# christopher-beckham/gan-heightmaps

Hardware: AMD Instinct MI355X
Metric: 512px heightmap+texture train images/sec (higher is better)
Workload: dtype bf16x3; 1 GPU; test1_nobn_bilin_both joint DCGAN+pix2pix train step (train_mode=both), 512x512, batch 4 per GPU, RMSprop lr 1e-4, LSGAN+100*L1; fp32 by operand splitting on the bf16 matrix cores (3 exact bf16 pieces per operand, 6 products, fp32 accumulation); global_batch=4, in_shp=512, parallelism=dp1, hip_graph=False, issue=recorded, streams=3

## Files before the change

gan_heightmaps_amd/_lib.py:

```python
import ctypes as C
import os

_HERE = os.path.dirname(os.path.abspath(__file__))
LIB_PATH = os.path.join(_HERE, "libghm.so")


class GhmError(RuntimeError):
    pass


class ConvDesc(C.Structure):
    _fields_ = [("N", C.c_int32), ("C", C.c_int32), ("H", C.c_int32), ("W", C.c_int32),
                ("K", C.c_int32), ("Ho", C.c_int32), ("Wo", C.c_int32),
                ("kh", C.c_int32), ("kw", C.c_int32), ("stride", C.c_int32), ("pad", C.c_int32),
                ("x_nstride", C.c_int64), ("y_nstride", C.c_int64)]


class RenderParams(C.Structure):
    _fields_ = [("pos", C.c_float * 3), ("yaw", C.c_float), ("pitch", C.c_float), ("fov", C.c_float),
                ("Hi", C.c_int32), ("Wi", C.c_int32),
                ("height_scale", C.c_float), ("step", C.c_float), ("max_dist", C.c_float),
                ("sun_azimuth", C.c_float), ("sun_elevation", C.c_float), ("shadows", C.c_int32),
                ("softness", C.c_float), ("ambient", C.c_float), ("haze", C.c_float),
                ("horizon", C.c_float * 3), ("zenith", C.c_float * 3), ("accel", C.c_int32), ("out_u8", C.c_int32)]
# ... 116 lines not shown
    "ghm_maxpool2_fwd": [_p, _p, _p, _i32, _i32, _i32, _i32],
    "ghm_maxpool2_bwd": [_p, _p, _p, _p, _p, _i32, _i32, _i32, _i32, _i32, _f],
    "ghm_avgpool_fwd": [_p, _p, _p, _i32, _i32, _i32, _i32, _i32],
    "ghm_avgpool_bwd": [_p, _p, _p, _i32, _i32, _i32, _i32, _i32],
    "ghm_dropout": [_p, _p, _i64, _p, _i64, _i32, _i32, _i32, _f, C.c_uint32, _p],
    "ghm_counter_tick": [_p, _p],
    "ghm_transpose_weights_batched": [_p, _p, _i32, _i32],
    "ghm_upconv_collapse_weights": [_p, _p, _p, _p, _p, _i32, _i32],
    "ghm_upconv_collapse_batched": [_p, _p, _i32, _i32],
    "ghm_upconv_expand_batched": [_p, _p, _i32, _i32, _i32],
    "ghm_blconv_frame_sizes": [_i32, _i32, _i32, _i32, _i32, C.POINTER(_i64), C.POINTER(_i64)],
    "ghm_blconv_frame_fwd": [_p, _p, _i64, _p, _p, _i64, _i32, _i32, _i32, _i32, _i32, _p],
    "ghm_blconv_frame_gather": [_p, _p, _i64, _i32, _i32, _i32, _i32, _i32, _p],
    "ghm_blconv_frame_dgrad": [_p, _p, _p, _p, _i64, _i32, _i32, _i32, _i32, _i32],
    "ghm_blconv_frame_wgrad": [_p, _p, _p, _p, _i32, _i32, _i32, _i32, _i32],
    "ghm_blconv_fwd_split": [_p, _D, _p, _i64, _i64, _p, _p, _p, _i32],
    "ghm_blconv_dgrad_split": [_p, _D, _p, _i64, _i64, _p, _p, _i32, _i32],
    "ghm_blconv_wgrad_split": [_p, _D, _p, _i64, _i64, _p, _i64, _i64, _p, _p, _i32, _i32],
    "ghm_upconv_expand_wgrad": [_p, _p, _p, _i32, _i32, _i32],
    "ghm_pp_to_hi": [_p, _p, _p, _i64, _i32, _i32, _i32, _i32],
    "ghm_hi_to_pp": [_p, _p, _i64, _p, _i32, _i32, _i32, _i32],
    "ghm_upsample_nearest2_fwd": [_p, _p, _i64, _p, _i32, _i32, _i32, _i32],
    "ghm_upsample_nearest2_bwd": [_p, _p, _p, _i64, _i32, _i32, _i32, _i32, _i32],
    "ghm_upsample_bilinear2_fwd": [_p, _p, _i64, _p, _i32, _i32, _i32, _i32],
    "ghm_upsample_bilinear2_bwd": [_p, _p, _p, _i64, _i32, _i32, _i32, _i32, _i32],
    "ghm_copy_view": [_p, _p, _i64, _p, _i64, _i32, _i32, _i32, _i32],
    "ghm_scale_samples": [_p, _p, _i64, _i32, _i32, _i32, _p, _i64, _p, _i64],
    "ghm_axpby": [_p, _f, _p, _f, _p, _i64],
    "ghm_image_batch": [_p, _p, _i32, _i32, _i32, _i32, _p, _i32, _p, _i64],
    "ghm_texture_gather": [_p, _p, _i32, _i32, _i32, _i32, _i32, _i32, _i32, _i32, _i32, _i32, _i32, _i32, _i32, _p, _i64],
# ... 128 lines not shown
```

gan_heightmaps_amd/csrc/conv_split.hip:

```cpp
#include <stdlib.h>
#include <string.h>

#include "common.h"

namespace {

typedef float f32x16 __attribute__((ext_vector_type(16)));
typedef float f32x2 __attribute__((ext_vector_type(2)));
typedef unsigned u32x4 __attribute__((ext_vector_type(4)));
typedef __bf16 bf16x8 __attribute__((ext_vector_type(8)));
typedef __bf16 bf16x2 __attribute__((ext_vector_type(2)));

__device__ __forceinline__ f32x16 sp_mfma(u32x4 a, u32x4 b, f32x16 c) {
    return __builtin_amdgcn_mfma_f32_32x32x16_bf16(__builtin_bit_cast(bf16x8, a), __builtin_bit_cast(bf16x8, b), c, 0, 0, 0);
}

__device__ __forceinline__ void sp_split2(float a, float b, unsigned& p0, unsigned& p1, unsigned& p2) {
    f32x2 v = {a, b};
    p0 = __builtin_bit_cast(unsigned, __builtin_convertvector(v, bf16x2));
    f32x2 r = {a - __uint_as_float(p0 << 16), b - __uint_as_float(p0 & 0xffff0000u)};
    p1 = __builtin_bit_cast(unsigned, __builtin_convertvector(r, bf16x2));
    f32x2 r2 = {r[0] - __uint_as_float(p1 << 16), r[1] - __uint_as_float(p1 & 0xffff0000u)};
    p2 = __builtin_bit_cast(unsigned, __builtin_convertvector(r2, bf16x2));
}
// ... 264 lines not shown
    static constexpr int PU1 = 2 * PH * PW, PCH = (PU1 + 63) / 64, PUP = PCH * 64;
    static constexpr int WU1 = 2 * KS * BM, NI = WU1 / 64;
    static constexpr int NW = WM * WN;
    static constexpr int NQ = (PCH + NW - 1) / NW;
    static constexpr int NIW = (NP * NI + NW - 1) / NW;
    static constexpr int WUNITS = NP * WU1, PUNITS = NP * PUP;
    static constexpr int SCR = 2 * WUNITS + 2 * PUNITS;
    static constexpr int LDS_BYTES = (SCR + 64 + 32) * 16;
};

template <int V>
struct SpIC {
    static constexpr int value = V;
};

template <int KS, int ST, int BM, int RT, int WM, int WN, bool POOL, int TW, int NP, int ABL = 0, int CLS = 0>
__global__ __launch_bounds__(WM * WN * 64, 1) void sp_conv2_kernel(const SpConvArgs a) {
    static_assert(CLS == 0 || (KS == 3 && ST == 1 && !POOL && ABL == 0), "class forms: 3x3 stride 1");
    typedef SpGeo2<KS, ST, BM, RT, WM, WN, TW, NP> G;
    typedef SpProd<NP> PR;
    constexpr int T = KS * KS;
    constexpr int RPF = G::RPF, ROWS = G::ROWS;
    constexpr int TM = BM / (WM * 32), TN = RT / WN;
    constexpr int PH = G::PH, PW = G::PW, PU1 = G::PU1, PCH = G::PCH, PUP = G::PUP;
    constexpr int PWE = (PW + 1) / 2;
    constexpr int WU1 = G::WU1, NI = G::NI, NW = G::NW, NQ = G::NQ, NIW = G::NIW;
    constexpr int WUNITS = G::WUNITS, PUNITS = G::PUNITS, SCR = G::SCR;
    constexpr int NMF = PR::N * TM * TN;
    constexpr int NRD = NP * (TM + TN);
    static_assert(TM >= 1 && TN >= 1 && KS >= 3, "tile / pipeline shape");
    extern __shared__ __attribute__((aligned(16))) u32x4 sp_smem[];
// ... 2 lines not shown
    u32x4* const Bl = sp_smem + SCR + 64;

    const int tid = threadIdx.x, lane = tid & 63, wave = __builtin_amdgcn_readfirstlane(tid >> 6);
    const int wm = wave / WN, wn = wave % WN;
    const int kg = lane >> 5, li = lane & 31;
    const int ntr = (a.R + BM - 1) / BM;
    const int tiles_x = a.W / TW, tiles_y = a.H / ROWS;
    const int lx = li % TW, ly = li / TW;
    const int HW = a.H * a.W, HWin = a.Hin * a.Win;
    const int nslabs = a.CH / 16;
    const int s_begin = blockIdx.y * a.slabs_per_split;
    const int s_end = min(nslabs, s_begin + a.slabs_per_split);
    struct Tile {
        int r0, n, y0, x0;
    };
    auto decode = [&](int v) {
        int L = CLS == 1 ? v : sp_xcd_remap(v, a.ntiles);
        Tile t;
        if (CLS == 1) {
            const int gs = a.cls_group, span = ntr * gs;
            const int g = L / span, rem = L - g * span;
            t.r0 = (rem / gs) * BM;
            L = g * gs + rem % gs;
        } else {
            t.r0 = (L % ntr) * BM;
            L /= ntr;
        }
        const int tx = L % tiles_x;
        L /= tiles_x;
        const int ty = L % tiles_y;
        t.n = L / tiles_y;
        t.y0 = ty * ROWS;
        t.x0 = tx * TW;
        return t;
    };
    int v = blockIdx.x;
    Tile tc = decode(v);
    const int cls1 = CLS == 1 ? tc.r0 / a.cls_k : 0;
    const int fa0 = CLS == 1 ? (cls1 >> 1) : 0, b0 = CLS == 1 ? (cls1 & 1) : 0;

    typedef const __attribute__((address_space(1))) void* gptr_t;
    typedef __attribute__((address_space(3))) void* lptr_t;

    const unsigned lane16 = lane * 16;
    unsigned wu[NIW];
    int wl[NIW];
    bool wreal[NIW];
    int wcol[NIW];
#pragma unroll
    for (int i = 0; i < NIW; ++i) {
        const int j = wave + i * NW;
        wreal[i] = j < NP * NI;
        const int jj = wreal[i] ? j : 0;
        const int p = jj / NI, w = jj - p * NI;
        const int ci = w / (BM / 64), h = w - ci * (BM / 64);
        const int cb = ci / KS, b = ci - cb * KS;
        wu[i] = (unsigned)(((long)p * a.wq_pstride + ((long)cb * T + b) * a.Rpad + h * 64) * 16);
        wl[i] = p * WU1 + w * 64;
        wcol[i] = b;
        if (CLS == 1 && b < b0) wreal[i] = false;
    }
    const long wrow = (long)KS * a.Rpad * 16;
    const long wslab = (long)2 * T * a.Rpad * 16;
    auto dma_w = [&](int r0, int s, int fa, int tog, int nc = KS) {
        const char* const src = (const char*)(a.wq + r0) + (long)s * wslab + fa * wrow;
#pragma unroll
        for (int i = 0; i < NIW; ++i)
            if (CLS != 0) {
                const bool real = wreal[i] && (CLS != 2 || wcol[i] < nc);
                __builtin_amdgcn_global_load_lds(real ? (gptr_t)(src + wu[i] + lane16) : (gptr_t)a.zeros,
                                                 (lptr_t)(sp_smem + (real ? wl[i] + tog : SCR)), 16, 0, 0);
            } else if (ABL & 16)
                __builtin_amdgcn_global_load_lds((gptr_t)(src + wu[i] + lane16), (lptr_t)(sp_smem + (wreal[i] ? wl[i] + tog : SCR)), 4, 0, 0);
            else if (ABL & 8)
                __builtin_amdgcn_global_load_lds((gptr_t)a.zeros, (lptr_t)(sp_smem + (wreal[i] ? wl[i] + tog : SCR)), 16, 0, 0);
            else
                __builtin_amdgcn_global_load_lds((gptr_t)(src + wu[i] + lane16), (lptr_t)(sp_smem + (wreal[i] ? wl[i] + tog : SCR)), 16, 0, 0);
    };

    const char* pp[NQ];
    unsigned pok = 0;
    int pcb[NQ], pyx[NQ];
    int pl[NQ];
    bool preal[NQ];
// ... 35 lines not shown
                    __builtin_amdgcn_global_load_lds((gptr_t)g, (lptr_t)(sp_smem + (preal[q] ? 2 * WUNITS + tog + p * PUP + pl[q] : SCR)), 4, 0, 0);
                else if (ABL & 8)
                    __builtin_amdgcn_global_load_lds((gptr_t)a.zeros, (lptr_t)(sp_smem + (preal[q] ? 2 * WUNITS + tog + p * PUP + pl[q] : SCR)), 16, 0, 0);
                else
                    __builtin_amdgcn_global_load_lds((gptr_t)g, (lptr_t)(sp_smem + (preal[q] ? 2 * WUNITS + tog + p * PUP + pl[q] : SCR)), 16, 0, 0);
                g += ok ? pstep : 0;
            }
        }
    };

    f32x16 acc[TM][TN], accc[TM][TN];

    struct Frag {
        u32x4 a[NP][TM], b[NP][TN];
    };
    const int wlane = kg * KS * BM + wm * (BM / WM) + li + b0 * BM;
    const int plane = kg * PH * PW + ((wn * TN * RPF + ly) * ST) * PW + (ST == 2 ? lx : lx * ST) + fa0 * PW + b0;
    auto rd = [&](Frag& f, const u32x4* Wb, const u32x4* Pb, int fa, int b) {
#pragma unroll
        for (int p = 0; p < NP; ++p) {
#pragma unroll
            for (int i = 0; i < TM; ++i) f.a[NP - 1 - p][i] = Wb[(NP - 1 - p) * WU1 + b * BM + i * 32];
#pragma unroll
            for (int j = 0; j < TN; ++j)
                f.b[p][j] = Pb[p * PUP + fa * PW + j * RPF * ST * PW + (ST == 2 ? (b & 1) * PWE + (b >> 1) : b)];
        }
    };
    auto mm = [&](const Frag& f) {
#pragma unroll
        for (int pr = 0; pr < PR::N; ++pr) {
#pragma unroll
            for (int i = 0; i < TM; ++i)
#pragma unroll
                for (int j = 0; j < TN; ++j) {
                    if (pr < PR::N - 1)
                        accc[i][j] = sp_mfma(f.a[PR::A[pr]][i], f.b[PR::B[pr]][j], accc[i][j]);
                    else
                        acc[i][j] = sp_mfma(f.a[0][i], f.b[0][j], acc[i][j]);
                }
        }
    };

    const int s_last = s_end - 1;
    auto ncols_of = [&](int s) { return CLS == 2 ? 3 - ((s / (a.cls_k / 16)) & 1) : KS; };
    if (s_begin < s_end) {
        dma_w(tc.r0, s_begin, fa0, 0, ncols_of(s_begin));
        dma_p(0, false);
    }
    asm volatile("s_waitcnt vmcnt(0)\n\ts_barrier" ::: "memory");
    if (s_begin < s_end) dma_w(tc.r0, s_begin, fa0 + 1, WUNITS, ncols_of(s_begin));
    int w0 = 0, p0 = 0;
    Frag cur;
    rd(cur, Wl + wlane, Pl + plane, 0, 0);

    for (;;) {
        const int vn = v + gridDim.x;
        const bool more = NW == 4 && CLS == 0 && vn < a.ntiles && s_begin < s_end;
        const Tile tn = decode(more ? vn : v);
#pragma unroll
        for (int i = 0; i < TM; ++i)
#pragma unroll
            for (int j = 0; j < TN; ++j)
#pragma unroll
                for (int e = 0; e < 16; ++e) acc[i][j][e] = accc[i][j][e] = 0.f;

        auto run = [&](auto NR_, auto NC_, int s_lo, int s_hi) {
            constexpr int NR = decltype(NR_)::value, NC = decltype(NC_)::value;
            static_assert(NR >= 2 && NC >= 2, "at least two filter rows / columns per slab");
            for (int s = s_lo; s < s_hi; ++s) {
                const bool last = s == s_last;
                const int sn = last ? (more ? s_begin : s) : s + 1;
                const int rn = (last && more) ? tn.r0 : tc.r0;
                const u32x4* const Pc = Pl + p0 + plane;
                const u32x4* const Pn = Pl + (PUNITS - p0) + plane;
#pragma unroll
                for (int fa = 0; fa < NR; ++fa) {
                    const int wc = (fa & 1) ? WUNITS - w0 : w0;
                    const u32x4* const Wc = Wl + wc + wlane;
                    const u32x4* const Wn = Wl + (WUNITS - wc) + wlane;
#pragma unroll
                    for (int b = 0; b < NC; ++b) {
                        Frag nx;
                        int ndma = 0;
                        if (ABL & 4) {
                            nx = cur;
                        } else if (b + 1 < NC) {
                            rd(nx, Wc, Pc, fa, b + 1);
                        } else {
                            rd(nx, Wn, fa + 1 < NR ? Pc : Pn, fa + 1 < NR ? fa + 1 : 0, 0);
                        }
                        if (b + 1 == NC && !(ABL & 1)) {
                            if (fa + 2 < NR)
                                dma_w(tc.r0, s, fa0 + fa + 2, wc, NC);
                            else
                                dma_w(rn, sn, fa0 + fa + 2 - NR, wc, ncols_of(sn));
                            ndma = NIW;
                        }
                        if (fa == 0 && b == 0 && !(ABL & 1)) {
                            if (last && more)
                                patch_of(tn);
                            dma_p(PUNITS - p0, !last);
                            ndma = NP * NQ;
                        }
                        mm(cur);
#pragma unroll
                        for (int m_ = 0; m_ < NRD; ++m_) {
                            __builtin_amdgcn_sched_group_barrier(0x008, 1, 0);
                            __builtin_amdgcn_sched_group_barrier(0x100, 1, 0);
                        }
#pragma unroll
// ... 24 lines not shown
                case 2: run(SpIC<2>{}, SpIC<3>{}, s_begin, s_end); break;
                default: run(SpIC<2>{}, SpIC<2>{}, s_begin, s_end); break;
            }
        } else {
            const int spc = a.cls_k / 16;
            run(SpIC<3>{}, SpIC<3>{}, max(s_begin, 0), min(s_end, spc));
            run(SpIC<3>{}, SpIC<2>{}, max(s_begin, spc), min(s_end, 2 * spc));
            run(SpIC<2>{}, SpIC<3>{}, max(s_begin, 2 * spc), min(s_end, 3 * spc));
            run(SpIC<2>{}, SpIC<2>{}, max(s_begin, 3 * spc), min(s_end, 4 * spc));
        }

        sp_conv_epilogue<BM, RT, WM, WN, POOL, TW, TM, TN, NP>(a, acc, accc, Bl, tid, wm, wn, kg, li, lx, ly, tc.n, tc.r0, tc.y0, tc.x0, HW);
        if (!more) break;
        v = vn;
        tc = tn;
    }
    asm volatile("s_waitcnt vmcnt(0)" ::: "memory");
}

struct SpWgradArgs {
    const u32x4* xq;
    long xq_ns, xq_ps;
    const u32x4* dyq;
    long dyq_ns, dyq_ps;
    const u32x4* zeros;
    float* out;
    int N, C, H, W, K, Ho, Wo;
    int rows_per_split, splits_per_col;
    long split_stride;
    int accumulate;
// ... 960 lines not shown
    for (int i = 0; i < nseen; ++i)
        if (seen[i] == (const void*)kernel) return 0;
    GHM_HIP(hipFuncSetAttribute((const void*)kernel, hipFuncAttributeMaxDynamicSharedMemorySize, 160 * 1024));
    if (nseen < 64) seen[nseen++] = (const void*)kernel;
    return 0;
}

template <int KS, int ST, int BM, int RT, int WM, int WN, bool POOL, int TW>
int sp_launch_variant(ghm_ctx* ctx, dim3 g, size_t lds, const SpConvArgs& a, int np, int cls = 0) {
    static_assert(SpGeo2<KS, ST, BM, RT, WM, WN, TW, 3>::LDS_BYTES <= 160 * 1024, "LDS");
    if (cls) {
        if constexpr (KS == 3 && ST == 1 && !POOL && TW == 32) {
#define GHM_CLS_CASE(NP_, C_)                                                                                                     \
            if constexpr (BM == 64 || C_ == 2)                                                                                    \
                if (np == NP_ && cls == C_) {                                                                                     \
                    if (int e = sp_set_lds(sp_conv2_kernel<KS, ST, BM, RT, WM, WN, POOL, TW, NP_, 0, C_>, lds)) return e;         \
                    hipLaunchKernelGGL((sp_conv2_kernel<KS, ST, BM, RT, WM, WN, POOL, TW, NP_, 0, C_>), g, dim3(WM * WN * 64), lds, \
                                       ctx->stream, a);                                                                           \
                    GHM_LAUNCH_CHECK();                                                                                           \
                    return 0;                                                                                                     \
                }
            GHM_CLS_CASE(3, 1) GHM_CLS_CASE(3, 2) GHM_CLS_CASE(2, 1) GHM_CLS_CASE(2, 2)
#undef GHM_CLS_CASE
        }
        ghm_set_error("split-fp32 convolution: no class form for this tile shape");
        return -3;
    }
#ifdef GHM_SPLIT_ABLATION
    if constexpr ((KS == 5 || (KS == 3 && ST == 1)) && BM == 64 && RT == 8 && !POOL && TW == 32) {
        const char* f = GHM_OPT("GHM_SPLIT_ABLATE");
        const int abl = f ? atoi(f) : 0;
#define GHM_ABL_CASE(A_)                                                                                              \
        if (abl == A_ && np == 3) {                                                                                   \
// ... 30 lines not shown
        void* ws = nullptr;
        if (int e = ghm_scratch(ctx, qbytes + pbytes, &ws)) return e;
        if (in32) {
            a.in_q = (const u32x4*)ws;
            a.in_q_nstride = (long)(a.CH / 8) * a.Hin * a.Win;
            a.in_q_pstride = plane;
            if (int e = sp_pack(ctx, in32, in32_nstride, a.N, a.CH, a.Hin * a.Win, ws, a.in_q_nstride, plane, NP)) return e;
        }
        if (pbytes) a.partial = (float*)((char*)ws + qbytes);
    }
    GHM_CHECK(!(pool && pl.splits > 1), "split-fp32 pooled convolution needs a single-pass plan");
    GHM_CHECK(!(a.out_q && pl.splits > 1), "split-fp32 convolution: a q output needs a single-pass plan (ask ghm_split_q_direct)");
    GHM_CHECK(pool || a.out || a.out_q, "split-fp32 convolution: no output");
    GHM_CHECK(!(a.accumulate && !a.out), "accumulate needs the fp32 output");
    GHM_CHECK(!a.out_q || (a.R % 8 == 0 && ((uintptr_t)a.out_q & 15) == 0), "q output: a multiple of 8 channels, 16-byte aligned");
    const dim3 g(cls ? pl.grid : pl.blocks, pl.splits);
    a.ntiles = pl.grid;
#define GHM_SP_CASE(KS_, ST_, BM_, RT_, WM_, WN_, POOL_, TW_)                                                    \
    if (ks == KS_ && st == ST_ && pl.bm == BM_ && pl.rt == RT_ && pl.wm == WM_ && pl.wn == WN_ && pool == POOL_ && pl.tw == TW_) {  \
        if (int e = sp_launch_variant<KS_, ST_, BM_, RT_, WM_, WN_, POOL_, TW_>(ctx, g, pl.lds, a, pl.np, cls)) return e;  \
    } else
    GHM_SP_CASE(5, 1, 64, 8, 1, 4, false, 32)
    GHM_SP_CASE(5, 1, 64, 8, 1, 4, true, 32)
    GHM_SP_CASE(3, 1, 128, 8, 2, 4, false, 32)
    GHM_SP_CASE(3, 1, 64, 8, 1, 4, false, 32)
    GHM_SP_CASE(3, 1, 128, 8, 2, 4, true, 32)
    GHM_SP_CASE(3, 1, 64, 8, 1, 4, true, 32)
    GHM_SP_CASE(3, 2, 64, 4, 2, 2, false, 32)
    GHM_SP_CASE(3, 2, 64, 4, 2, 4, false, 32)
    GHM_SP_CASE(5, 1, 64, 4, 2, 2, false, 16)
    GHM_SP_CASE(3, 1, 64, 4, 2, 2, false, 16)
// ... 418 lines not shown
    if (d->stride == 2)
        return sp_dgrad_s2(ctx, d, dy, dyq, dyq_nstride, dyq_pstride, wqT, bias, dx, act, alpha, accumulate, nullptr, 0, 0.f, dxq,
                           (long)dxq_nstride, pieces);
    const SpPlan pl = sp_plan(d->N, d->K, d->H, d->W, d->C, d->kh, 1, ctx->num_cu, pieces);
    SpConvArgs a;
    memset(&a, 0, sizeof(a));
    a.in_q = (const u32x4*)dyq; a.in_q_nstride = dyq_nstride; a.in_q_pstride = dyq_pstride;
    a.wq = (const u32x4*)wqT; a.bias = bias; a.out = dx; a.out_q = (uint2*)dxq; a.out_q_nstride = dxq_nstride;
    a.N = d->N; a.CH = d->K; a.H = d->H; a.W = d->W; a.Hin = d->H; a.Win = d->W;
    a.R = d->C; a.Rpad = sp_rpad(d->C); a.wq_pstride = (long)sp_nblk(d->K) * d->kh * d->kw * a.Rpad;
    a.out_nstride = d->x_nstride; a.pad = d->kh - 1 - d->pad;
    a.act = act; a.alpha = alpha; a.accumulate = accumulate;
    return sp_launch_conv(ctx, pl, a, d->kh, 1, dyq ? nullptr : dy, d->y_nstride, false);
}

int ghm_blconv_split_supported(const ghm_conv_desc* d, int32_t kind) {
    if (!d || d->kh != 3 || d->kw != 3 || d->stride != 1 || d->pad != 1 || d->K % 4 || GHM_OPT("GHM_BLCONV_NO_SKIP")) return 0;
    const int ck = d->K / 4;
    if (ck % 64) return 0;
    if (kind == 0) {
        const SpPlan pl = sp_plan(d->N, d->C, d->Ho, d->Wo, d->K, 3, 1, ghm_plan_cus(), 3, true);
        return sp_fwd_geom(d) && pl.ok && pl.tw == 32 && pl.bm == 64;
    }
    if (kind == 1) {
        const SpPlan pl = sp_plan(d->N, d->K, d->H, d->W, d->C, 3, 1, ghm_plan_cus(), 3, GHM_OPT("GHM_BLCONV_DGRAD_BM64") != nullptr);
        return sp_fwd_geom(d) && pl.ok && pl.tw == 32;
    }
    if (kind == 2) {
        const SpWPlan v = sp_wplan(d, ghm_plan_cus());
        return v.ok && v.cht == 2 && v.ct == 2 && v.spx == 32;
    }
    return 0;
}

int ghm_blconv_fwd_split(ghm_ctx* ctx, const ghm_conv_desc* d, const void* xq, int64_t xq_nstride, int64_t xq_pstride, const void* wq,
                         const float* bias, float* y, int32_t pieces) {
    GHM_CHECK(ctx && d && xq && wq && y, "null argument");
    GHM_SP_PIECES_OK(pieces);
    GHM_CHECK(ghm_blconv_split_supported(d, 0), "ghm_blconv_fwd_split: geometry not served (ask ghm_blconv_split_supported)");
    const int ck = d->K / 4;
    const SpPlan pl = sp_plan(d->N, d->C, d->Ho, d->Wo, d->K, 3, 1, ctx->num_cu, pieces, true);
    SpConvArgs a;
    memset(&a, 0, sizeof(a));
    a.in_q = (const u32x4*)xq; a.in_q_nstride = xq_nstride; a.in_q_pstride = xq_pstride;
    a.wq = (const u32x4*)wq; a.bias = bias; a.out = y;
    a.N = d->N; a.CH = d->C; a.H = d->Ho; a.W = d->Wo; a.Hin = d->H; a.Win = d->W;
    a.R = d->K; a.Rpad = sp_rpad(d->K); a.wq_pstride = (long)sp_nblk(d->C) * 9 * a.Rpad;
    a.out_nstride = d->y_nstride; a.pad = 1;
    a.act = GHM_ACT_LINEAR; a.cls_k = ck;
    {
        const int per = pl.grid / ((d->K + pl.bm - 1) / pl.bm), ntr = (d->K + pl.bm - 1) / pl.bm;
        int gs = 8;
        while (gs * 2 * ntr <= 2 * ctx->num_cu && per % (gs * 2) == 0) gs *= 2;
        if (per % gs) gs = per;
        if (const char* f = GHM_OPT("GHM_BLCONV_GROUP")) gs = (atoi(f) > 0 && per % atoi(f) == 0) ? atoi(f) : per;
        a.cls_group = gs;
    }
    SpPlan p2 = pl;
    const int nslabs = d->C / 16;
    if (p2.splits == 1 && p2.grid <= ctx->num_cu && nslabs >= 16 && !GHM_OPT("GHM_BLCONV_NO_SPLITK")) {
        p2.splits = 2;
        p2.slabs_per_split = (nslabs + 1) / 2;
    }
    return sp_launch_conv(ctx, p2, a, 3, 1, nullptr, 0, false, 1);
}

int ghm_blconv_dgrad_split(ghm_ctx* ctx, const ghm_conv_desc* d, const void* dyq, int64_t dyq_nstride, int64_t dyq_pstride,
                           const void* wqT, float* dx, int32_t accumulate, int32_t pieces) {
    GHM_CHECK(ctx && d && dyq && wqT && dx, "null argument");
    GHM_SP_PIECES_OK(pieces);
    GHM_CHECK(ghm_blconv_split_supported(d, 1), "ghm_blconv_dgrad_split: geometry not served (ask ghm_blconv_split_supported)");
    const SpPlan pl = sp_plan(d->N, d->K, d->H, d->W, d->C, 3, 1, ctx->num_cu, pieces, GHM_OPT("GHM_BLCONV_DGRAD_BM64") != nullptr);
    SpConvArgs a;
    memset(&a, 0, sizeof(a));
    a.in_q = (const u32x4*)dyq; a.in_q_nstride = dyq_nstride; a.in_q_pstride = dyq_pstride;
    a.wq = (const u32x4*)wqT; a.out = dx;
    a.N = d->N; a.CH = d->K; a.H = d->H; a.W = d->W; a.Hin = d->H; a.Win = d->W;
    a.R = d->C; a.Rpad = sp_rpad(d->C); a.wq_pstride = (long)sp_nblk(d->K) * 9 * a.Rpad;
    a.out_nstride = d->x_nstride; a.pad = 1;
    a.act = GHM_ACT_LINEAR; a.accumulate = accumulate; a.cls_k = d->K / 4;
    return sp_launch_conv(ctx, pl, a, 3, 1, nullptr, 0, false, 2);
}

int ghm_blconv_wgrad_split(ghm_ctx* ctx, const ghm_conv_desc* d, const void* xq, int64_t xq_nstride, int64_t xq_pstride,
                           const void* dyq, int64_t dyq_nstride, int64_t dyq_pstride, float* dwp, void* workspace,
                           int32_t accumulate, int32_t pieces) {
    GHM_CHECK(ctx && d && xq && dyq && dwp, "null argument");
// ... 38 lines not shown
```

gan_heightmaps_amd/device.py:

```python
import ctypes as C

import numpy as np

from . import _lib
from ._lib import ConvDesc, call

ACT_CODES = {'linear': 0, 'relu': 1, 'lrelu': 2, 'sigmoid': 3, 'tanh': 4}
DTYPE_CODES = {'f32': 0, 'bf16': 1, 'f16': 2}
SPLIT = 'bf16x3'
DTYPE_CODES[SPLIT] = 3
SPLIT2 = 'bf16x2'
DTYPE_CODES[SPLIT2] = 4
SPLITS = {SPLIT: 3, SPLIT2: 2}


def device_count():
    n = C.c_int32(0)
    call("ghm_device_count", C.byref(n))
    return n.value


class DevTensor:
    __slots__ = ("dev", "ptr", "shape", "nstride", "base")

# ... 438 lines not shown

    def blconv_frame_fwd(self, x, wp, y_pp, K, FL):
        call("ghm_blconv_frame_fwd", self.h, _vp(x), x.nstride, _vp(wp), _vp(y_pp), y_pp.nstride, x.N, x.Cc, int(K), x.H, x.W, _vp(FL))

    def blconv_frame_gather(self, dy_pp, Cc, K, DYL):
        call("ghm_blconv_frame_gather", self.h, _vp(dy_pp), dy_pp.nstride, dy_pp.N, int(Cc), int(K), dy_pp.H, dy_pp.W, _vp(DYL))

    def blconv_frame_dgrad(self, DYL, wp, dx, K):
        call("ghm_blconv_frame_dgrad", self.h, _vp(DYL), _vp(wp), _vp(dx), dx.nstride, dx.N, dx.Cc, int(K), dx.H, dx.W)

    def blconv_frame_wgrad(self, DYL, FL, dwp, N, Cc, K, n1, n2):
        call("ghm_blconv_frame_wgrad", self.h, _vp(DYL), _vp(FL), _vp(dwp), int(N), int(Cc), int(K), int(n1), int(n2))

    def blconv_split_supported(self, d, kind, dtype):
        return dtype in SPLITS and bool(_lib.load().ghm_blconv_split_supported(C.byref(d), int(kind)))

    def blconv_fwd_split(self, d, xq, wq, bias, y, dtype):
        call("ghm_blconv_fwd_split", self.h, C.byref(d), C.c_void_p(xq.ptr), xq.nstride, xq.pstride, _vp(wq), _vp(bias), _vp(y),
             SPLITS[dtype])

    def blconv_dgrad_split(self, d, dyq, wqT, dx, dtype, accumulate=False):
        call("ghm_blconv_dgrad_split", self.h, C.byref(d), C.c_void_p(dyq.ptr), dyq.nstride, dyq.pstride, _vp(wqT), _vp(dx),
             int(accumulate), SPLITS[dtype])

    def blconv_wgrad_split(self, d, xq, dyq, dwp, ws, dtype, accumulate=False):
        call("ghm_blconv_wgrad_split", self.h, C.byref(d), C.c_void_p(xq.ptr), xq.nstride, xq.pstride, C.c_void_p(dyq.ptr),
             dyq.nstride, dyq.pstride, _vp(dwp), _vp(ws), int(accumulate), SPLITS[dtype])

    def transpose_table(self, items):
        rec = np.zeros(len(items), dtype=[('wp', '<u8'), ('wpT', '<u8'), ('C', '<i4'), ('T', '<i4'), ('K', '<i4'),
# ... 689 lines not shown
```

include/ghm.h:

```cpp
#ifndef GHM_H
#define GHM_H

#include <stddef.h>
#include <stdint.h>

#ifdef __cplusplus
extern "C" {
#endif

typedef struct ghm_ctx ghm_ctx;
typedef struct ghm_graph ghm_graph;
typedef struct ghm_step ghm_step;

enum { GHM_DTYPE_F32 = 0, GHM_DTYPE_BF16 = 1, GHM_DTYPE_F16 = 2 };

enum { GHM_ACT_LINEAR = 0, GHM_ACT_RELU = 1, GHM_ACT_LRELU = 2, GHM_ACT_SIGMOID = 3, GHM_ACT_TANH = 4 };

typedef struct {
    int32_t N;
    int32_t C, H, W;
    int32_t K, Ho, Wo;
    int32_t kh, kw, stride, pad;
    int64_t x_nstride;
    int64_t y_nstride;
// ... 193 lines not shown
int ghm_upconv_collapse_weights(ghm_ctx* ctx, const float* wp5, const float* bias, float* wpc, float* bias4, int32_t C, int32_t K);
int ghm_upconv_collapse_batched(ghm_ctx* ctx, const void* table, int32_t n_items, int32_t total_blocks);
int ghm_upconv_expand_wgrad(ghm_ctx* ctx, const float* dwpc, float* dwp5, int32_t C, int32_t K, int32_t accumulate);
int ghm_upconv_expand_batched(ghm_ctx* ctx, const void* table, int32_t n_items, int32_t total_blocks, int32_t accumulate);
int ghm_blconv_supported(int32_t N, int32_t C, int32_t K, int32_t n1, int32_t n2);
int ghm_blconv_frame_sizes(int32_t N, int32_t C, int32_t K, int32_t n1, int32_t n2, int64_t* fl_floats, int64_t* dyl_floats);
int ghm_blconv_frame_fwd(ghm_ctx* ctx, const float* x, int64_t x_nstride, const float* wp, float* y_pp, int64_t y_nstride, int32_t N,
                         int32_t C, int32_t K, int32_t n1, int32_t n2, float* FL);
int ghm_blconv_frame_gather(ghm_ctx* ctx, const float* dy_pp, int64_t dy_nstride, int32_t N, int32_t C, int32_t K, int32_t n1,
                            int32_t n2, float* DYL);
int ghm_blconv_frame_dgrad(ghm_ctx* ctx, const float* DYL, const float* wp, float* dx, int64_t dx_nstride, int32_t N, int32_t C,
                           int32_t K, int32_t n1, int32_t n2);
int ghm_blconv_frame_wgrad(ghm_ctx* ctx, const float* DYL, const float* FL, float* dwp, int32_t N, int32_t C, int32_t K, int32_t n1,
                           int32_t n2);
int ghm_blconv_split_supported(const ghm_conv_desc* d, int32_t kind);
int ghm_blconv_fwd_split(ghm_ctx* ctx, const ghm_conv_desc* d, const void* xq, int64_t xq_nstride, int64_t xq_pstride, const void* wq,
                         const float* bias, float* y, int32_t pieces);
int ghm_blconv_dgrad_split(ghm_ctx* ctx, const ghm_conv_desc* d, const void* dyq, int64_t dyq_nstride, int64_t dyq_pstride,
                           const void* wqT, float* dx, int32_t accumulate, int32_t pieces);
int ghm_blconv_wgrad_split(ghm_ctx* ctx, const ghm_conv_desc* d, const void* xq, int64_t xq_nstride, int64_t xq_pstride,
                           const void* dyq, int64_t dyq_nstride, int64_t dyq_pstride, float* dwp, void* workspace,
                           int32_t accumulate, int32_t pieces);
int ghm_pp_to_hi(ghm_ctx* ctx, const float* pp, float* hi, int64_t hi_nstride, int32_t N, int32_t K, int32_t H, int32_t W);
int ghm_hi_to_pp(ghm_ctx* ctx, const float* hi, int64_t hi_nstride, float* pp, int32_t N, int32_t K, int32_t H, int32_t W);
int ghm_upsample_bilinear2_fwd(ghm_ctx* ctx, const float* x, int64_t x_nstride, float* y, int32_t N, int32_t C, int32_t H, int32_t W);
int ghm_upsample_bilinear2_bwd(ghm_ctx* ctx, const float* dy, float* dx, int64_t dx_nstride, int32_t N, int32_t C, int32_t H, int32_t W, int32_t accumulate);
int ghm_copy_view(ghm_ctx* ctx, const float* x, int64_t x_nstride, float* y, int64_t y_nstride, int32_t N, int32_t C, int32_t HW, int32_t accumulate);
int ghm_scale_samples(ghm_ctx* ctx, float* x, int64_t x_nstride, int32_t N, int32_t C, int32_t HW, const float* num, int64_t num_nstride,
                      const float* den, int64_t den_nstride);
int ghm_axpby(ghm_ctx* ctx, float a, const float* x, float b, float* y, int64_t n);
// ... 183 lines not shown
```

Before: 314.2 images/s.

## Make class-form bilinear-conv split kernels persistent with balanced tail partitioning

Class-form (CLS==1) 3x3 split-fp32 conv kernels for the bilinear-upsample conv path now run persistently when the plan has fewer blocks than tiles. Each block walks a contiguous run of tiles, covering all four phase classes per spatial/filter unit, and the remainder units are split across 2 or 4 blocks to balance the tail. Per-tile class offsets (weight/patch LDS offsets, first filter row, column skip) become runtime and are handed to the prefetch of the next tile, so the pipeline carries across tiles. The dgrad planner may pick BM=64 to enable this. Planning logic is factored out and exposed via a new query entry point, with an env switch to disable persistence. The intent is less launch-wave quantization and lower prologue cost, at the price of more register and address arithmetic.

```diff
diff --git a/gan_heightmaps_amd/_lib.py b/gan_heightmaps_amd/_lib.py
--- a/gan_heightmaps_amd/_lib.py
+++ b/gan_heightmaps_amd/_lib.py
@@ -154,6 +154,7 @@
     "ghm_blconv_frame_gather": [_p, _p, _i64, _i32, _i32, _i32, _i32, _i32, _p],
     "ghm_blconv_frame_dgrad": [_p, _p, _p, _p, _i64, _i32, _i32, _i32, _i32, _i32],
     "ghm_blconv_frame_wgrad": [_p, _p, _p, _p, _i32, _i32, _i32, _i32, _i32],
+    "ghm_blconv_split_plan": [_D, _i32, _i32, C.POINTER(_i32)],
     "ghm_blconv_fwd_split": [_p, _D, _p, _i64, _i64, _p, _p, _p, _i32],
     "ghm_blconv_dgrad_split": [_p, _D, _p, _i64, _i64, _p, _p, _i32, _i32],
     "ghm_blconv_wgrad_split": [_p, _D, _p, _i64, _i64, _p, _i64, _i64, _p, _p, _i32, _i32],
diff --git a/gan_heightmaps_amd/csrc/conv_split.hip b/gan_heightmaps_amd/csrc/conv_split.hip
--- a/gan_heightmaps_amd/csrc/conv_split.hip
+++ b/gan_heightmaps_amd/csrc/conv_split.hip
@@ -302,7 +302,7 @@
     static constexpr int value = V;
 };
 
-template <int KS, int ST, int BM, int RT, int WM, int WN, bool POOL, int TW, int NP, int ABL = 0, int CLS = 0>
+template <int KS, int ST, int BM, int RT, int WM, int WN, bool POOL, int TW, int NP, int ABL = 0, int CLS = 0, bool PST = true>
 __global__ __launch_bounds__(WM * WN * 64, 1) void sp_conv2_kernel(const SpConvArgs a) {
     static_assert(CLS == 0 || (KS == 3 && ST == 1 && !POOL && ABL == 0), "class forms: 3x3 stride 1");
     typedef SpGeo2<KS, ST, BM, RT, WM, WN, TW, NP> G;
@@ -335,10 +335,32 @@
     struct Tile {
         int r0, n, y0, x0;
     };
+    const bool sb_on = PST && CLS == 1 && a.cls_group == 0;
+    const int sb_fpc = CLS == 1 ? a.cls_k / BM : 1;
+    const int sb_units = tiles_x * tiles_y * a.N * sb_fpc;
+    const int sb_full = sb_units / (int)gridDim.x, sb_rem = sb_units - sb_full * (int)gridDim.x;
+    const int sb_parts = sb_rem == 0 ? 1 : ((int)gridDim.x >= 4 * sb_rem ? 4 : ((int)gridDim.x >= 2 * sb_rem ? 2 : 1));
+    const bool sb_tail = (int)blockIdx.x < sb_parts * sb_rem;
+    const int sb_steps = 4 * sb_full + (sb_tail ? 4 / sb_parts : 0);
+    const int sb_lf = sp_xcd_remap(blockIdx.x, gridDim.x);
+    const int sb_lt = sb_tail ? sp_xcd_remap(blockIdx.x, sb_parts * sb_rem) : 0;
+    if (sb_on && sb_steps == 0) return;
     auto decode = [&](int v) {
         int L = CLS == 1 ? v : sp_xcd_remap(v, a.ntiles);
         Tile t;
-        if (CLS == 1) {
+        if (sb_on) {
+            int u, c;
+            if (v < 4 * sb_full) {
+                u = (v >> 2) * (int)gridDim.x + sb_lf;
+                c = v & 3;
+            } else {
+                const int j = v - 4 * sb_full, part = sb_lt % sb_parts;
+                u = sb_full * (int)gridDim.x + sb_lt / sb_parts;
+                c = sb_parts == 1 ? j : (sb_parts == 2 ? (j ? 3 - part : part) : part);
+            }
+            L = u / sb_fpc;
+            t.r0 = (c * sb_fpc + (u - L * sb_fpc)) * BM;
+        } else if (CLS == 1) {
             const int gs = a.cls_group, span = ntr * gs;
             const int g = L / span, rem = L - g * span;
             t.r0 = (rem / gs) * BM;
@@ -355,10 +377,12 @@
         t.x0 = tx * TW;
         return t;
     };
-    int v = blockIdx.x;
+    int v = sb_on ? 0 : blockIdx.x;
     Tile tc = decode(v);
-    const int cls1 = CLS == 1 ? tc.r0 / a.cls_k : 0;
-    const int fa0 = CLS == 1 ? (cls1 >> 1) : 0, b0 = CLS == 1 ? (cls1 & 1) : 0;
+    int cls1 = CLS == 1 ? tc.r0 / a.cls_k : 0;
+    int fa0 = CLS == 1 ? (cls1 >> 1) : 0, b0 = CLS == 1 ? (cls1 & 1) : 0;
+    int woff = b0 * BM, poff = fa0 * PW + b0;
+    int cls1n = cls1, fa0n = fa0, b0n = b0, woffn = woff, poffn = poff;
 
     typedef const __attribute__((address_space(1))) void* gptr_t;
     typedef __attribute__((address_space(3))) void* lptr_t;
@@ -367,7 +391,7 @@
     unsigned wu[NIW];
     int wl[NIW];
     bool wreal[NIW];
-    int wcol[NIW];
+    unsigned m_all = 0, m_no0 = 0, m_no2 = 0;
 #pragma unroll
     for (int i = 0; i < NIW; ++i) {
         const int j = wave + i * NW;
@@ -378,17 +402,19 @@
         const int cb = ci / KS, b = ci - cb * KS;
         wu[i] = (unsigned)(((long)p * a.wq_pstride + ((long)cb * T + b) * a.Rpad + h * 64) * 16);
         wl[i] = p * WU1 + w * 64;
-        wcol[i] = b;
-        if (CLS == 1 && b < b0) wreal[i] = false;
+        m_all |= wreal[i] ? 1u << i : 0u;
+        m_no0 |= (wreal[i] && b >= 1) ? 1u << i : 0u;
+        m_no2 |= (wreal[i] && b < 2) ? 1u << i : 0u;
     }
     const long wrow = (long)KS * a.Rpad * 16;
     const long wslab = (long)2 * T * a.Rpad * 16;
-    auto dma_w = [&](int r0, int s, int fa, int tog, int nc = KS) {
+    auto dma_w = [&](int r0, int s, int fa, int tog, int nc = KS, int c0 = 0) {
         const char* const src = (const char*)(a.wq + r0) + (long)s * wslab + fa * wrow;
+        const unsigned mask = CLS == 1 ? (c0 ? m_no0 : m_all) : (nc == 2 ? m_no2 : m_all);
 #pragma unroll
         for (int i = 0; i < NIW; ++i)
             if (CLS != 0) {
-                const bool real = wreal[i] && (CLS != 2 || wcol[i] < nc);
+                const bool real = (mask >> i) & 1u;
                 __builtin_amdgcn_global_load_lds(real ? (gptr_t)(src + wu[i] + lane16) : (gptr_t)a.zeros,
                                                  (lptr_t)(sp_smem + (real ? wl[i] + tog : SCR)), 16, 0, 0);
             } else if (ABL & 16)
@@ -454,8 +480,8 @@
     struct Frag {
         u32x4 a[NP][TM], b[NP][TN];
     };
-    const int wlane = kg * KS * BM + wm * (BM / WM) + li + b0 * BM;
-    const int plane = kg * PH * PW + ((wn * TN * RPF + ly) * ST) * PW + (ST == 2 ? lx : lx * ST) + fa0 * PW + b0;
+    const int wlane = kg * KS * BM + wm * (BM / WM) + li;
+    const int plane = kg * PH * PW + ((wn * TN * RPF + ly) * ST) * PW + (ST == 2 ? lx : lx * ST);
     auto rd = [&](Frag& f, const u32x4* Wb, const u32x4* Pb, int fa, int b) {
 #pragma unroll
         for (int p = 0; p < NP; ++p) {
@@ -484,19 +510,26 @@
     const int s_last = s_end - 1;
     auto ncols_of = [&](int s) { return CLS == 2 ? 3 - ((s / (a.cls_k / 16)) & 1) : KS; };
     if (s_begin < s_end) {
-        dma_w(tc.r0, s_begin, fa0, 0, ncols_of(s_begin));
+        dma_w(tc.r0, s_begin, fa0, 0, ncols_of(s_begin), b0);
         dma_p(0, false);
     }
     asm volatile("s_waitcnt vmcnt(0)\n\ts_barrier" ::: "memory");
-    if (s_begin < s_end) dma_w(tc.r0, s_begin, fa0 + 1, WUNITS, ncols_of(s_begin));
+    if (s_begin < s_end) dma_w(tc.r0, s_begin, fa0 + 1, WUNITS, ncols_of(s_begin), b0);
     int w0 = 0, p0 = 0;
     Frag cur;
-    rd(cur, Wl + wlane, Pl + plane, 0, 0);
+    rd(cur, Wl + wlane + woff, Pl + plane + poff, 0, 0);
 
     for (;;) {
-        const int vn = v + gridDim.x;
-        const bool more = NW == 4 && CLS == 0 && vn < a.ntiles && s_begin < s_end;
+        const int vn = sb_on ? v + 1 : v + (int)gridDim.x;
+        const bool more = PST && NW == 4 && (sb_on ? vn < sb_steps : vn < a.ntiles) && s_begin < s_end;
         const Tile tn = decode(more ? vn : v);
+        if (CLS == 1) {
+            cls1n = tn.r0 / a.cls_k;
+            fa0n = cls1n >> 1;
+            b0n = cls1n & 1;
+            woffn = b0n * BM;
+            poffn = fa0n * PW + b0n;
+        }
 #pragma unroll
         for (int i = 0; i < TM; ++i)
 #pragma unroll
@@ -510,14 +543,16 @@
             for (int s = s_lo; s < s_hi; ++s) {
                 const bool last = s == s_last;
                 const int sn = last ? (more ? s_begin : s) : s + 1;
-                const int rn = (last && more) ? tn.r0 : tc.r0;
-                const u32x4* const Pc = Pl + p0 + plane;
-                const u32x4* const Pn = Pl + (PUNITS - p0) + plane;
+                const bool hand = last && more;
+                const int rn = hand ? tn.r0 : tc.r0;
+                const int fan = (CLS == 1 && hand) ? fa0n : fa0, bn = (CLS == 1 && hand) ? b0n : b0;
+                const u32x4* const Pc = Pl + p0 + plane + poff;
+                const u32x4* const Pn = Pl + (PUNITS - p0) + plane + ((CLS == 1 && hand) ? poffn : poff);
 #pragma unroll
                 for (int fa = 0; fa < NR; ++fa) {
                     const int wc = (fa & 1) ? WUNITS - w0 : w0;
-                    const u32x4* const Wc = Wl + wc + wlane;
-                    const u32x4* const Wn = Wl + (WUNITS - wc) + wlane;
+                    const u32x4* const Wc = Wl + wc + wlane + woff;
+                    const u32x4* const Wn = Wl + (WUNITS - wc) + wlane + ((CLS == 1 && hand && fa + 1 == NR) ? woffn : woff);
 #pragma unroll
                     for (int b = 0; b < NC; ++b) {
                         Frag nx;
@@ -531,9 +566,9 @@
                         }
                         if (b + 1 == NC && !(ABL & 1)) {
                             if (fa + 2 < NR)
-                                dma_w(tc.r0, s, fa0 + fa + 2, wc, NC);
+                                dma_w(tc.r0, s, fa0 + fa + 2, wc, NC, b0);
                             else
-                                dma_w(rn, sn, fa0 + fa + 2 - NR, wc, ncols_of(sn));
+                                dma_w(rn, sn, fan + fa + 2 - NR, wc, ncols_of(sn), bn);
                             ndma = NIW;
                         }
                         if (fa == 0 && b == 0 && !(ABL & 1)) {
@@ -588,6 +623,9 @@
         if (!more) break;
         v = vn;
         tc = tn;
+        if (CLS == 1) {
+            cls1 = cls1n; fa0 = fa0n; b0 = b0n; woff = woffn; poff = poffn;
+        }
     }
     asm volatile("s_waitcnt vmcnt(0)" ::: "memory");
 }
@@ -1578,9 +1616,15 @@
 #define GHM_CLS_CASE(NP_, C_)                                                                                                     \
             if constexpr (BM == 64 || C_ == 2)                                                                                    \
                 if (np == NP_ && cls == C_) {                                                                                     \
-                    if (int e = sp_set_lds(sp_conv2_kernel<KS, ST, BM, RT, WM, WN, POOL, TW, NP_, 0, C_>, lds)) return e;         \
-                    hipLaunchKernelGGL((sp_conv2_kernel<KS, ST, BM, RT, WM, WN, POOL, TW, NP_, 0, C_>), g, dim3(WM * WN * 64), lds, \
-                                       ctx->stream, a);                                                                           \
+                    if (BM == 64 && (int)g.x < a.ntiles) {                                                 \
+                        if (int e = sp_set_lds(sp_conv2_kernel<KS, ST, BM, RT, WM, WN, POOL, TW, NP_, 0, C_, BM == 64>, lds)) return e; \
+                        hipLaunchKernelGGL((sp_conv2_kernel<KS, ST, BM, RT, WM, WN, POOL, TW, NP_, 0, C_, BM == 64>), g,          \
+                                           dim3(WM * WN * 64), lds, ctx->stream, a);                                              \
+                    } else {                                                                                                      \
+                        if (int e = sp_set_lds(sp_conv2_kernel<KS, ST, BM, RT, WM, WN, POOL, TW, NP_, 0, C_, false>, lds)) return e; \
+                        hipLaunchKernelGGL((sp_conv2_kernel<KS, ST, BM, RT, WM, WN, POOL, TW, NP_, 0, C_, false>), g,             \
+                                           dim3(WM * WN * 64), lds, ctx->stream, a);                                              \
+                    }                                                                                                             \
                     GHM_LAUNCH_CHECK();                                                                                           \
                     return 0;                                                                                                     \
                 }
@@ -1641,7 +1685,7 @@
     GHM_CHECK(pool || a.out || a.out_q, "split-fp32 convolution: no output");
     GHM_CHECK(!(a.accumulate && !a.out), "accumulate needs the fp32 output");
     GHM_CHECK(!a.out_q || (a.R % 8 == 0 && ((uintptr_t)a.out_q & 15) == 0), "q output: a multiple of 8 channels, 16-byte aligned");
-    const dim3 g(cls ? pl.grid : pl.blocks, pl.splits);
+    const dim3 g(pl.blocks, pl.splits);
     a.ntiles = pl.grid;
 #define GHM_SP_CASE(KS_, ST_, BM_, RT_, WM_, WN_, POOL_, TW_)                                                    \
     if (ks == KS_ && st == ST_ && pl.bm == BM_ && pl.rt == RT_ && pl.wm == WM_ && pl.wn == WN_ && pool == POOL_ && pl.tw == TW_) {  \
@@ -2090,16 +2134,62 @@
     return sp_launch_conv(ctx, pl, a, d->kh, 1, dyq ? nullptr : dy, d->y_nstride, false);
 }
 
+static bool sp_blconv_persist() { return GHM_OPT("GHM_BLCONV_NO_PERSIST") == nullptr; }
+
+static SpPlan sp_plan_blconv_fwd(const ghm_conv_desc* d, int num_cu, int np, int* group) {
+    SpPlan pl = sp_plan(d->N, d->C, d->Ho, d->Wo, d->K, 3, 1, num_cu, np, true);
+    if (!pl.ok) return pl;
+    const int nslabs = d->C / 16;
+    if (pl.splits == 1 && pl.grid <= num_cu && nslabs >= 16 && !GHM_OPT("GHM_BLCONV_NO_SPLITK")) {
+        pl.splits = 2;
+        pl.slabs_per_split = (nslabs + 1) / 2;
+    }
+    if (pl.splits > 1 || !sp_blconv_persist()) pl.blocks = pl.grid;
+    int gs = 0;
+    if (pl.blocks == pl.grid) {
+        const int ntr = (d->K + pl.bm - 1) / pl.bm, per = pl.grid / ntr;
+        gs = 8;
+        while (gs * 2 * ntr <= 2 * num_cu && per % (gs * 2) == 0) gs *= 2;
+        if (per % gs) gs = per;
+        if (const char* f = GHM_OPT("GHM_BLCONV_GROUP")) gs = (atoi(f) > 0 && per % atoi(f) == 0) ? atoi(f) : per;
+    }
+    if (group) *group = gs;
+    return pl;
+}
+
+static SpPlan sp_plan_blconv_dgrad(const ghm_conv_desc* d, int num_cu, int np) {
+    SpPlan pl = sp_plan(d->N, d->K, d->H, d->W, d->C, 3, 1, num_cu, np, GHM_OPT("GHM_BLCONV_DGRAD_BM64") != nullptr);
+    if (!sp_blconv_persist()) {
+        pl.blocks = pl.grid;
+        return pl;
+    }
+    if (pl.ok && pl.bm == 128) {
+        const SpPlan p64 = sp_plan(d->N, d->K, d->H, d->W, d->C, 3, 1, num_cu, np, true);
+        if (p64.ok && p64.tw == 32 && p64.splits == 1 && p64.blocks < p64.grid && p64.grid >= 2 * p64.blocks) pl = p64;
+    }
+    return pl;
+}
+
+int ghm_blconv_split_plan(const ghm_conv_desc* d, int32_t kind, int32_t pieces, int32_t* out) {
+    GHM_CHECK(d && out && (kind == 0 || kind == 1), "ghm_blconv_split_plan: descriptor, forward or data gradient, six ints");
+    GHM_SP_PIECES_OK(pieces);
+    GHM_CHECK(ghm_blconv_split_supported(d, kind), "ghm_blconv_split_plan: geometry not served (ask ghm_blconv_split_supported)");
+    int gs = 0;
+    const SpPlan pl = kind == 0 ? sp_plan_blconv_fwd(d, ghm_plan_cus(), pieces, &gs) : sp_plan_blconv_dgrad(d, ghm_plan_cus(), pieces);
+    out[0] = pl.bm; out[1] = pl.grid; out[2] = pl.blocks; out[3] = pl.splits; out[4] = pl.slabs_per_split; out[5] = gs;
+    return 0;
+}
+
 int ghm_blconv_split_supported(const ghm_conv_desc* d, int32_t kind) {
     if (!d || d->kh != 3 || d->kw != 3 || d->stride != 1 || d->pad != 1 || d->K % 4 || GHM_OPT("GHM_BLCONV_NO_SKIP")) return 0;
     const int ck = d->K / 4;
     if (ck % 64) return 0;
     if (kind == 0) {
-        const SpPlan pl = sp_plan(d->N, d->C, d->Ho, d->Wo, d->K, 3, 1, ghm_plan_cus(), 3, true);
+        const SpPlan pl = sp_plan_blconv_fwd(d, ghm_plan_cus(), 3, nullptr);
         return sp_fwd_geom(d) && pl.ok && pl.tw == 32 && pl.bm == 64;
     }
     if (kind == 1) {
-        const SpPlan pl = sp_plan(d->N, d->K, d->H, d->W, d->C, 3, 1, ghm_plan_cus(), 3, GHM_OPT("GHM_BLCONV_DGRAD_BM64") != nullptr);
+        const SpPlan pl = sp_plan_blconv_dgrad(d, ghm_plan_cus(), 3);
         return sp_fwd_geom(d) && pl.ok && pl.tw == 32;
     }
     if (kind == 2) {
@@ -2115,7 +2205,8 @@
     GHM_SP_PIECES_OK(pieces);
     GHM_CHECK(ghm_blconv_split_supported(d, 0), "ghm_blconv_fwd_split: geometry not served (ask ghm_blconv_split_supported)");
     const int ck = d->K / 4;
-    const SpPlan pl = sp_plan(d->N, d->C, d->Ho, d->Wo, d->K, 3, 1, ctx->num_cu, pieces, true);
+    int gs = 0;
+    const SpPlan pl = sp_plan_blconv_fwd(d, ctx->num_cu, pieces, &gs);
     SpConvArgs a;
     memset(&a, 0, sizeof(a));
     a.in_q = (const u32x4*)xq; a.in_q_nstride = xq_nstride; a.in_q_pstride = xq_pstride;
@@ -2124,21 +2215,8 @@
     a.R = d->K; a.Rpad = sp_rpad(d->K); a.wq_pstride = (long)sp_nblk(d->C) * 9 * a.Rpad;
     a.out_nstride = d->y_nstride; a.pad = 1;
     a.act = GHM_ACT_LINEAR; a.cls_k = ck;
-    {
-        const int per = pl.grid / ((d->K + pl.bm - 1) / pl.bm), ntr = (d->K + pl.bm - 1) / pl.bm;
-        int gs = 8;
-        while (gs * 2 * ntr <= 2 * ctx->num_cu && per % (gs * 2) == 0) gs *= 2;
-        if (per % gs) gs = per;
-        if (const char* f = GHM_OPT("GHM_BLCONV_GROUP")) gs = (atoi(f) > 0 && per % atoi(f) == 0) ? atoi(f) : per;
-        a.cls_group = gs;
-    }
-    SpPlan p2 = pl;
-    const int nslabs = d->C / 16;
-    if (p2.splits == 1 && p2.grid <= ctx->num_cu && nslabs >= 16 && !GHM_OPT("GHM_BLCONV_NO_SPLITK")) {
-        p2.splits = 2;
-        p2.slabs_per_split = (nslabs + 1) / 2;
-    }
-    return sp_launch_conv(ctx, p2, a, 3, 1, nullptr, 0, false, 1);
+    a.cls_group = gs;
+    return sp_launch_conv(ctx, pl, a, 3, 1, nullptr, 0, false, 1);
 }
 
 int ghm_blconv_dgrad_split(ghm_ctx* ctx, const ghm_conv_desc* d, const void* dyq, int64_t dyq_nstride, int64_t dyq_pstride,
@@ -2146,7 +2224,7 @@
     GHM_CHECK(ctx && d && dyq && wqT && dx, "null argument");
     GHM_SP_PIECES_OK(pieces);
     GHM_CHECK(ghm_blconv_split_supported(d, 1), "ghm_blconv_dgrad_split: geometry not served (ask ghm_blconv_split_supported)");
-    const SpPlan pl = sp_plan(d->N, d->K, d->H, d->W, d->C, 3, 1, ctx->num_cu, pieces, GHM_OPT("GHM_BLCONV_DGRAD_BM64") != nullptr);
+    const SpPlan pl = sp_plan_blconv_dgrad(d, ctx->num_cu, pieces);
     SpConvArgs a;
     memset(&a, 0, sizeof(a));
     a.in_q = (const u32x4*)dyq; a.in_q_nstride = dyq_nstride; a.in_q_pstride = dyq_pstride;
diff --git a/gan_heightmaps_amd/device.py b/gan_heightmaps_amd/device.py
--- a/gan_heightmaps_amd/device.py
+++ b/gan_heightmaps_amd/device.py
@@ -476,6 +476,11 @@
 
     def blconv_split_supported(self, d, kind, dtype):
         return dtype in SPLITS and bool(_lib.load().ghm_blconv_split_supported(C.byref(d), int(kind)))
+
+    def blconv_split_plan(self, d, kind, dtype):
+        out = (C.c_int32 * 6)()
+        call("ghm_blconv_split_plan", C.byref(d), int(kind), SPLITS[dtype], out)
+        return dict(zip(("bm", "tiles", "blocks", "splits", "slabs_per_split", "group"), (int(v) for v in out)))
 
     def blconv_fwd_split(self, d, xq, wq, bias, y, dtype):
         call("ghm_blconv_fwd_split", self.h, C.byref(d), C.c_void_p(xq.ptr), xq.nstride, xq.pstride, _vp(wq), _vp(bias), _vp(y),
diff --git a/include/ghm.h b/include/ghm.h
--- a/include/ghm.h
+++ b/include/ghm.h
@@ -231,6 +231,7 @@
 int ghm_blconv_frame_wgrad(ghm_ctx* ctx, const float* DYL, const float* FL, float* dwp, int32_t N, int32_t C, int32_t K, int32_t n1,
                            int32_t n2);
 int ghm_blconv_split_supported(const ghm_conv_desc* d, int32_t kind);
+int ghm_blconv_split_plan(const ghm_conv_desc* d, int32_t kind, int32_t pieces, int32_t* out);
 int ghm_blconv_fwd_split(ghm_ctx* ctx, const ghm_conv_desc* d, const void* xq, int64_t xq_nstride, int64_t xq_pstride, const void* wq,
                          const float* bias, float* y, int32_t pieces);
 int ghm_blconv_dgrad_split(ghm_ctx* ctx, const ghm_conv_desc* d, const void* dyq, int64_t dyq_nstride, int64_t dyq_pstride,
```

New measurement: 315.7 images/s, median of 6. No clear change (+0.5%).
